# gongweibao/FleetX

Measured on AMD Instinct MI355X. Metric: tokens/sec (whole node) GPT-3 6.7B hybrid-parallel at 1/2/4/8 MI355X, higher is better.
Workload: dtype bf16; 1 GPU; model=gpt3-6.7B, global_batch=8, seq_len=1024, parallelism=dp1, micro_batch=8, hip_graph=True, grad_reduce_dtype=float32, recompute=False

## Files before the change

### csrc/kernels/bindings.cpp

```cpp
#include <hip/hip_runtime.h>
#include <pybind11/pybind11.h>
#include <pybind11/stl.h>
#include <stdint.h>
#include <string>
#include <stdexcept>
#include <vector>

namespace py = pybind11;
typedef uintptr_t ptr;

#include "fx_api.h"

#define P(x) reinterpret_cast<void*>(x)
#define CP(x) reinterpret_cast<const void*>(x)
#define S(x) reinterpret_cast<hipStream_t>(x)
#define F(x) reinterpret_cast<float*>(x)

static std::vector<long> v3(const std::vector<long>& a) {
  std::vector<long> r(a);
  r.resize(3, 0);
  return r;
}

PYBIND11_MODULE(_kernels, m) {
  m.doc() = "FleetX-AMD HIP kernels (gfx950)";
  m.def("coltile_splits", &fx_coltile_splits);
  m.def("add_ln_fwd", [](int dt, ptr x, ptr bias, ptr res, ptr g, ptr b, ptr s_out, ptr y,
                         ptr mean, ptr rstd, int rows, int h, float eps, float p, uint64_t key,
                         ptr salt, ptr st) {
    fx_add_ln_fwd(dt, CP(x), CP(bias), CP(res), CP(g), CP(b), P(s_out), P(y), F(mean), F(rstd),
                  rows, h, eps, p, key, CP(salt), S(st));
  });
  m.def("ln_bwd_row", [](int dt, ptr dy, ptr s, ptr mean, ptr rstd, ptr g, ptr ds_in, ptr ds_out,
                         ptr dx_out, int rows, int h, float p, uint64_t key, ptr salt, ptr st) {
    fx_ln_bwd_row(dt, CP(dy), CP(s), F(mean), F(rstd), CP(g), CP(ds_in), P(ds_out), P(dx_out),
                  rows, h, p, key, CP(salt), S(st));
  });
  m.def("ln_bwd_cols_blocks", &fx_ln_bwd_cols_blocks);
  m.def("ln_bwd_cols", [](int dt, ptr dy, ptr s, ptr mean, ptr rstd, ptr g, ptr ds_in, ptr ds_out,
                          ptr dx_out, int rows, int h, float p, uint64_t key, ptr part,
                          int with_dbias, ptr fg, ptr tg, int accg, ptr fb, ptr tb, int accb,
                          ptr fx, ptr tx, int accx, ptr salt, ptr st) {
    return fx_ln_bwd_cols(dt, CP(dy), CP(s), F(mean), F(rstd), CP(g), CP(ds_in), P(ds_out),
                          P(dx_out), rows, h, p, key, F(part), with_dbias, F(fg), P(tg), accg,
                          F(fb), P(tb), accb, F(fx), P(tx), accx, CP(salt), S(st));
  }, py::arg("dt"), py::arg("dy"), py::arg("s"), py::arg("mean"), py::arg("rstd"), py::arg("g"),
     py::arg("ds_in"), py::arg("ds_out"), py::arg("dx_out"), py::arg("rows"), py::arg("h"),
     py::arg("p"), py::arg("key"), py::arg("part"), py::arg("with_dbias"), py::arg("fg") = 0,
     py::arg("tg") = 0, py::arg("accg") = 0, py::arg("fb") = 0, py::arg("tb") = 0,
     py::arg("accb") = 0, py::arg("fx") = 0, py::arg("tx") = 0, py::arg("accx") = 0,
     py::arg("salt") = 0, py::arg("st") = 0);
  m.def("coltile_partial", [](int dt, int mode, ptr a, ptr b, ptr mean, ptr rstd, ptr p0, ptr p1,
                              int rows, int cols, int splits, ptr st, ptr cnt, ptr f0, ptr t0,
                              int acc0, ptr f1, ptr t1, int acc1) {
    fx_coltile_partial(dt, mode, CP(a), CP(b), F(mean), F(rstd), F(p0), F(p1), rows, cols, splits,
                       S(st), reinterpret_cast<int*>(cnt), F(f0), P(t0), acc0, F(f1), P(t1),
                       acc1);
  }, py::arg("dt"), py::arg("mode"), py::arg("a"), py::arg("b"), py::arg("mean"), py::arg("rstd"),
     py::arg("p0"), py::arg("p1"), py::arg("rows"), py::arg("cols"), py::arg("splits"),
     py::arg("st"), py::arg("cnt") = 0, py::arg("f0") = 0, py::arg("t0") = 0, py::arg("acc0") = 0,
     py::arg("f1") = 0, py::arg("t1") = 0, py::arg("acc1") = 0);
  m.def("coltile_finalize", [](int dt, ptr part, int splits, int cols, ptr out_f32, ptr out_t,
                               int accumulate, ptr st) {
    fx_coltile_finalize(dt, F(part), splits, cols, F(out_f32), P(out_t), accumulate, S(st));
  });
  m.def("bias_gelu_fwd", [](int dt, int erf, ptr x, ptr bias, ptr y, long n, int cols, ptr st) {
    fx_bias_gelu_fwd(dt, erf, CP(x), CP(bias), P(y), n, cols, S(st));
  });
  m.def("bias_gelu_bwd", [](int dt, int erf, ptr dy, ptr x, ptr bias, ptr dx, ptr part, int rows,
                            int cols, int splits, ptr st, ptr cnt, ptr out_f32, ptr out_t,
                            int acc) {
    fx_bias_gelu_bwd(dt, erf, CP(dy), CP(x), CP(bias), P(dx), F(part), rows, cols, splits, S(st),
                     reinterpret_cast<int*>(cnt), F(out_f32), P(out_t), acc);
  }, py::arg("dt"), py::arg("erf"), py::arg("dy"), py::arg("x"), py::arg("bias"), py::arg("dx"),
// ... 238 lines not shown
```

### csrc/kernels/fx_api.h

```cpp
#pragma once
#include <hip/hip_runtime.h>
#include <stdint.h>

extern "C" {
int fx_coltile_splits(int rows, int cols);
void fx_add_ln_fwd(int, const void*, const void*, const void*, const void*, const void*, void*,
                   void*, float*, float*, int, int, float, float, uint64_t, const void*,
                   hipStream_t);
void fx_ln_bwd_row(int, const void*, const void*, const float*, const float*, const void*,
                   const void*, void*, void*, int, int, float, uint64_t, const void*, hipStream_t);
int fx_ln_bwd_cols_blocks(int, int, int);
int fx_ln_bwd_cols(int, const void*, const void*, const float*, const float*, const void*,
                   const void*, void*, void*, int, int, float, uint64_t, float*, int, float*, void*,
                   int, float*, void*, int, float*, void*, int, const void*, hipStream_t);
void fx_coltile_partial(int, int, const void*, const void*, const float*, const float*, float*,
                        float*, int, int, int, hipStream_t, int*, float*, void*, int, float*,
                        void*, int);
void fx_coltile_finalize(int, const float*, int, int, float*, void*, int, hipStream_t);
void fx_bias_gelu_fwd(int, int, const void*, const void*, void*, long, int, hipStream_t);
void fx_bias_gelu_bwd(int, int, const void*, const void*, const void*, void*, float*, int, int, int,
                      hipStream_t, int*, float*, void*, int);
void fx_bias_dropout_add_fwd(int, const void*, const void*, const void*, void*, long, int, float,
                             uint64_t, const void*, hipStream_t);
void fx_dropout_bwd_colsum(int, const void*, void*, float*, int, int, int, float, uint64_t,
                           const void*, hipStream_t, int*, float*, void*, int);
void fx_dropout_fwd(int, const void*, void*, long, float, uint64_t, const void*, hipStream_t);
void fx_ce_stats(int, const void*, const int64_t*, int, int, long, float*, float*, float*, int,
                 hipStream_t);
void fx_ce_bwd(int, const void*, void*, const int64_t*, const float*, const float*, int, int, long,
               int, hipStream_t);
int fx_sumsq_blocks(long n);
void fx_sumsq_f32(const float*, long, float*, int, hipStream_t);
void fx_sumsq_16(int, const void*, long, float*, int, hipStream_t);
void fx_sumsq_chunks(const int64_t*, const int64_t*, int, float*, hipStream_t);
int fx_adamw(int dtype, int flags, void* master, const void* grad, float* m, float* v, void* p16,
             long n, float lr, float beta1, float beta2, float eps, float wd, float l2,
             const float* gscale, const int* skip, const int* step, const float* lr_dev,
// ... 75 lines not shown
```

### csrc/kernels/layout.hip

```cpp
#include "fx_api.h"
#include "fx_common.h"

namespace {

constexpr int TR = 64, TC = 256;
constexpr int TPAD = 2;

template <typename T, bool COLSUM>
__global__ __launch_bounds__(256) void transpose16_kernel(const uint16_t* __restrict__ x,
                                                          uint16_t* __restrict__ y,
                                                          float* __restrict__ part, int R, int C,
                                                          long ldx, long ldy, int tiles_c) {
  __shared__ uint16_t t[TR][TC + TPAD];
  const int bc = blockIdx.x % tiles_c;
  const int br = blockIdx.x / tiles_c;
  const int r0 = br * TR, c0 = bc * TC;
  const int tid = threadIdx.x;
  uint4 v[8];
#pragma unroll
  for (int k = 0; k < 8; ++k) {
    const int r = (tid >> 5) + 8 * k, cc = (tid & 31) * 8;
    if (r0 + r < R && c0 + cc < C)
      v[k] = *reinterpret_cast<const uint4*>(x + (long)(r0 + r) * ldx + c0 + cc);
    else
      v[k] = make_uint4(0, 0, 0, 0);
  }
#pragma unroll
  for (int k = 0; k < 8; ++k) {
    const int r = (tid >> 5) + 8 * k, cc = (tid & 31) * 8;
    uint32_t* d = reinterpret_cast<uint32_t*>(&t[r][cc]);
    d[0] = v[k].x;
    d[1] = v[k].y;
    d[2] = v[k].z;
    d[3] = v[k].w;
  }
  __syncthreads();
#pragma unroll
  for (int k = 0; k < 8; ++k) {
    const int id = tid + k * 256;
    const int c = id >> 3, rr = (id & 7) * 8;
    uint16_t h[8];
#pragma unroll
    for (int i = 0; i < 8; ++i) h[i] = t[rr + i][c];
    if (c0 + c < C && r0 + rr < R)
      *reinterpret_cast<uint4*>(y + (long)(c0 + c) * ldy + r0 + rr) =
          *reinterpret_cast<const uint4*>(h);
    if constexpr (COLSUM) {
      float s = 0.f;
#pragma unroll
      for (int i = 0; i < 8; ++i) s += Elt<T>::to_f(h[i]);
      s += __shfl_xor(s, 1, 64);
      s += __shfl_xor(s, 2, 64);
      s += __shfl_xor(s, 4, 64);
      if ((id & 7) == 0 && c0 + c < C) part[(long)br * C + c0 + c] = s;
    }
  }
}

}

extern "C" int fx_transpose16(int dtype, const void* x, void* y, float* part, int R, int C,
                              long ldx, long ldy, hipStream_t st) {
  if ((R | C) & 7 || ldx & 7 || ldy & 7) return -1;
  if (R == 0 || C == 0) return 0;
  const int tiles_c = (C + TC - 1) / TC;
  const long blocks = (long)tiles_c * ((R + TR - 1) / TR);
  if (blocks > 0x7fffffffL) return -2;
// ... 12 lines not shown
```

### csrc/kernels/norm_eltwise.hip

```cpp
#include "fx_api.h"
#include "fx_common.h"

namespace {

struct DropCfg {
  uint32_t klo, khi, thr;
  float scale;
  int enabled;
  const uint64_t* salt;
};

__device__ __forceinline__ DropCfg resolve_drop(DropCfg d) {
  if (d.enabled && d.salt != nullptr) {
    const uint64_t k = salt_key(((uint64_t)d.khi << 32) | d.klo, *d.salt);
    d.klo = (uint32_t)k;
    d.khi = (uint32_t)(k >> 32);
  }
  return d;
}

__device__ __forceinline__ float drop_apply(float v, uint64_t idx, const DropCfg& d) {
  if (!d.enabled) return v;
  uint32_t h = elem_rand_pair(idx, d.klo, d.khi);
  uint32_t r = (idx & 1) ? (h >> 16) : (h & 0xffffu);
  return r >= d.thr ? v * d.scale : 0.f;
}

__device__ __forceinline__ void drop_apply8(float* v, uint64_t idx0, const DropCfg& d) {
  if (!d.enabled) return;
#pragma unroll
  for (int q = 0; q < 4; ++q) {
    const uint32_t h = elem_rand_pair(idx0 + 2 * q, d.klo, d.khi);
// ... 195 lines not shown
#pragma unroll
    for (int i = 0; i < VPT; ++i) {
      const int c = (i * 64 + lane) * 8;
      dr[i] = make_uint4(0, 0, 0, 0);
      if (!MASK || c < h) dr[i] = *reinterpret_cast<const uint4*>(ds_in + base + c);
    }
  }
  const float m1 = wave_sum(s1) / h, m2 = wave_sum(s2) / h;
#pragma unroll
  for (int i = 0; i < VPT; ++i) {
    const int c = (i * 64 + lane) * 8;
    if (MASK && c >= h) continue;
    float o[8];
#pragma unroll
    for (int j = 0; j < 8; ++j) o[j] = rstd * (gdy[i][j] - m1 - xh[i][j] * m2);
    if (ds_in) {
      float r[8];
      unpack8<T>(dr[i], r);
#pragma unroll
      for (int j = 0; j < 8; ++j) o[j] += r[j];
    }
    store8<T>(ds_out + base + c, o);
    if (drop.enabled) {
      drop_apply8(o, base + c, drop);
      store8<T>(dx_out + base + c, o);
    } else if (dx_out != ds_out) {
      store8<T>(dx_out + base + c, o);
    }
  }
}

template <typename T>
__global__ __launch_bounds__(256) void ln_bwd_row_generic(
    const uint16_t* __restrict__ dy, const uint16_t* __restrict__ s,
    const float* __restrict__ mean_in, const float* __restrict__ rstd_in,
    const uint16_t* __restrict__ gamma, const uint16_t* __restrict__ ds_in,
    uint16_t* __restrict__ ds_out, uint16_t* __restrict__ dx_out, int rows, int h,
    DropCfg drop_) {
  const DropCfg drop = resolve_drop(drop_);
  const int lane = threadIdx.x & 63;
  const int row = blockIdx.x * 4 + (threadIdx.x >> 6);
  if (row >= rows) return;
  const size_t base = (size_t)row * h;
  const float mean = mean_in[row], rstd = rstd_in[row];
  const int nv = h / 8;
  float s1 = 0.f, s2 = 0.f;
// ... 3 lines not shown
    load8<T>(gamma + vi * 8, g);
    load8<T>(dy + base + vi * 8, d);
    for (int j = 0; j < 8; ++j) {
      float xh = (a[j] - mean) * rstd, gd = d[j] * g[j];
      s1 += gd;
      s2 += gd * xh;
    }
  }
  const float m1 = wave_sum(s1) / h, m2 = wave_sum(s2) / h;
  for (int vi = lane; vi < nv; vi += 64) {
    const int c = vi * 8;
    float a[8], g[8], d[8], o[8];
    load8<T>(s + base + c, a);
    load8<T>(gamma + c, g);
    load8<T>(dy + base + c, d);
    for (int j = 0; j < 8; ++j) o[j] = rstd * (d[j] * g[j] - m1 - (a[j] - mean) * rstd * m2);
    if (ds_in) {
      float r[8];
      load8<T>(ds_in + base + c, r);
      for (int j = 0; j < 8; ++j) o[j] += r[j];
    }
    store8<T>(ds_out + base + c, o);
    if (drop.enabled) {
      drop_apply8(o, base + c, drop);
      store8<T>(dx_out + base + c, o);
    } else if (dx_out != ds_out) {
      store8<T>(dx_out + base + c, o);
    }
  }
}

template <typename T, int VPT, int WPR, bool MASK, bool DB>
__global__ __launch_bounds__(256, 2) void ln_bwd_cols_kernel(
    const uint16_t* __restrict__ dy, const uint16_t* __restrict__ s,
    const float* __restrict__ mean_in, const float* __restrict__ rstd_in,
    const uint16_t* __restrict__ gamma, const uint16_t* __restrict__ ds_in,
    uint16_t* __restrict__ ds_out, uint16_t* __restrict__ dx_out, int rows, int h,
    int rows_per_group, float* __restrict__ part, DropCfg drop_) {
  constexpr int NG = 4 / WPR;
  __shared__ float red[4 * 512 * VPT];
  __shared__ float xs[2][4][2];
  const DropCfg drop = resolve_drop(drop_);
  const int lane = threadIdx.x & 63, w = threadIdx.x >> 6;
  const int grp = w / WPR, half = w % WPR;
  const int hw = h / WPR, cbase = half * hw;
  const int r0 = min(rows, (blockIdx.x * NG + grp) * rows_per_group);
// ... 70 lines not shown
        s2 += xs[k & 1][WPR * grp + q][1];
      }
    }
    if (!live) continue;
    const float m1 = s1 / h, m2 = s2 / h;
#pragma unroll
    for (int i = 0; i < VPT; ++i) {
      const int c = (i * 64 + lane) * 8;
      if (MASK && c >= hw) continue;
      float a[8], d[8], g[8], o[8];
      unpack8<T>(ca[i], a);
      unpack8<T>(cd[i], d);
      unpack8<T>(gp[i], g);
#pragma unroll
      for (int j = 0; j < 8; ++j) o[j] = rstd * (d[j] * g[j] - m1 - (a[j] - mean) * rstd * m2);
      if (ds_in) {
        float rr[8];
        unpack8<T>(cr[i], rr);
#pragma unroll
        for (int j = 0; j < 8; ++j) o[j] += rr[j];
      }
      store8<T>(ds_out + base + c, o);
      if (drop.enabled) {
        drop_apply8(o, base + c, drop);
        store8<T>(dx_out + base + c, o);
      } else if (dx_out != ds_out) {
        store8<T>(dx_out + base + c, o);
      }
      if (DB) {
#pragma unroll
        for (int j = 0; j < 8; ++j) ax[i][j] += round_to<T>(o[j]);
      }
    }
  }
#pragma unroll
  for (int arr = 0; arr < (DB ? 3 : 2); ++arr) {
    __syncthreads();
#pragma unroll
    for (int i = 0; i < VPT; ++i) {
      const int c = (i * 64 + lane) * 8;
      if (MASK && c >= hw) continue;
#pragma unroll
      for (int j = 0; j < 8; ++j)
        red[grp * h + cbase + c + j] = arr == 0 ? ag[i][j] : arr == 1 ? ab[i][j] : ax[DB ? i : 0][j];
    }
    __syncthreads();
// ... 241 lines not shown
  const int col = blockIdx.x * 128 + tx * 8;
  const int r0 = blockIdx.y * rows_per_split;
  const int r1 = min(rows, r0 + rows_per_split);
  float acc[8];
#pragma unroll
  for (int j = 0; j < 8; ++j) acc[j] = 0.f;
  if (col < cols) {
    float b[8];
    if (bias) load8<T>(bias + col, b);
    else {
#pragma unroll
      for (int j = 0; j < 8; ++j) b[j] = 0.f;
    }
    for (int r = r0 + ty; r < r1; r += 16) {
      const size_t off = (size_t)r * cols + col;
      float g[8], a[8];
      load8<T>(dy + off, g);
      load8<T>(x + off, a);
#pragma unroll
      for (int j = 0; j < 8; ++j) {
        float t = a[j] + b[j];
        g[j] *= ERF ? gelu_erf_grad(t) : gelu_tanh_grad(t);
      }
      store8<T>(dx + off, g);
#pragma unroll
      for (int j = 0; j < 8; ++j) acc[j] += round_to<T>(g[j]);
    }
  }
#pragma unroll
  for (int j = 0; j < 8; ++j) red[ty][tx * 8 + j] = acc[j];
  __syncthreads();
  if (threadIdx.x < 128) {
    float s = 0.f;
#pragma unroll
    for (int t = 0; t < 16; ++t) s += red[t][threadIdx.x];
    const int gc = blockIdx.x * 128 + threadIdx.x;
    if (part && gc < cols) st_part(part + (size_t)blockIdx.y * cols + gc, s);
  }
  if (fin.cnt) colsum_tail<T>(part, nullptr, cols, 1, fin);
}

template <typename T>
__global__ __launch_bounds__(256) void bias_dropout_add_fwd_kernel(
    const uint16_t* __restrict__ x, const uint16_t* __restrict__ bias,
    const uint16_t* __restrict__ residual, uint16_t* __restrict__ out, long n8, int cols,
    DropCfg drop_) {
// ... 85 lines not shown
                                                          DropCfg drop_) {
  const DropCfg drop = resolve_drop(drop_);
  const long n8 = n / 8;
  for (long v = blockIdx.x * (long)blockDim.x + threadIdx.x; v < n8; v += (long)gridDim.x * blockDim.x) {
    const long off = v * 8;
    float a[8];
    load8<T>(x + off, a);
    drop_apply8(a, (uint64_t)off, drop);
    store8<T>(y + off, a);
  }
  for (long i = n8 * 8 + blockIdx.x * (long)blockDim.x + threadIdx.x; i < n;
       i += (long)gridDim.x * blockDim.x)
    y[i] = Elt<T>::from_f(drop_apply(Elt<T>::to_f(x[i]), (uint64_t)i, drop));
}

DropCfg make_drop(float p, uint64_t key, const void* salt) {
  DropCfg d;
  d.enabled = p > 0.f ? 1 : 0;
  d.klo = (uint32_t)(key & 0xffffffffu);
  d.khi = (uint32_t)(key >> 32);
  d.thr = (uint32_t)(p * 65536.0f + 0.5f);
  d.scale = p < 1.f ? 1.f / (1.f - p) : 0.f;
  d.salt = reinterpret_cast<const uint64_t*>(salt);
  return d;
}

inline int grid_for(long n8) {
  long g = (n8 + 255) / 256;
  if (g > 8192) g = 8192;
  if (g < 1) g = 1;
  return (int)g;
}

inline int splits_for(int rows, int cols) {
  static const int blocks = [] {
    const char* e = getenv("FLEETX_COLSUM_BLOCKS");
    const int v = e ? atoi(e) : 0;
    return v > 0 ? v : 1024;
  }();
  int tiles = (cols + 127) / 128;
  int s = blocks / (tiles > 0 ? tiles : 1);
  if (s < 1) s = 1;
  int max_s = (rows + 15) / 16;
  if (s > max_s) s = max_s;
  if (s > 512) s = 512;
  return s;
// ... 48 lines not shown
                                 X, B, R, G, Be, S, Y, mean, rstd, rows, h, eps, d));
    }
  } else if (h % 8 == 0 && h < 8 * 512) {
#define LNM_CASE(V)                                                                          \
  case V:                                                                                    \
    FX_DISPATCH_T(dtype, add_ln_fwd_kernel<T, V, true><<<grid, block, 0, st>>>(              \
                             X, B, R, G, Be, S, Y, mean, rstd, rows, h, eps, d));            \
    break;
    switch ((h + 511) / 512) {
      LNM_CASE(1) LNM_CASE(2) LNM_CASE(3) LNM_CASE(4) LNM_CASE(5) LNM_CASE(6) LNM_CASE(7)
      LNM_CASE(8)
    }
#undef LNM_CASE
  } else {
    FX_DISPATCH_T(dtype, add_ln_fwd_generic<T><<<grid, block, 0, st>>>(
                             X, B, R, G, Be, S, Y, mean, rstd, rows, h, eps, d));
  }
#undef LN_CASE
}

extern "C" void fx_ln_bwd_row(int dtype, const void* dy, const void* s, const float* mean,
                              const float* rstd, const void* gamma, const void* ds_in,
                              void* ds_out, void* dx_out, int rows, int h, float p, uint64_t key,
                              const void* salt, hipStream_t st) {
  DropCfg d = make_drop(p, key, salt);
  dim3 grid((rows + 3) / 4), block(256);
  auto DY = (const uint16_t*)dy;
  auto S = (const uint16_t*)s;
  auto G = (const uint16_t*)gamma;
  auto DI = (const uint16_t*)ds_in;
  auto DS = (uint16_t*)ds_out;
  auto DX = (uint16_t*)dx_out;
#define LNB_CASE(V)                                                                       \
  case V:                                                                                 \
    FX_DISPATCH_T(dtype, ln_bwd_row_kernel<T, V><<<grid, block, 0, st>>>(                 \
                             DY, S, mean, rstd, G, DI, DS, DX, rows, h, d));              \
    break;
  if (h % 512 == 0 && h / 512 <= 8) {
    switch (h / 512) {
      LNB_CASE(1) LNB_CASE(2) LNB_CASE(3) LNB_CASE(4) LNB_CASE(5) LNB_CASE(6) LNB_CASE(7)
      LNB_CASE(8)
      default:
        FX_DISPATCH_T(dtype, ln_bwd_row_generic<T><<<grid, block, 0, st>>>(
                                 DY, S, mean, rstd, G, DI, DS, DX, rows, h, d));
    }
  } else if (h % 8 == 0 && h < 8 * 512) {
#define LNBM_CASE(V)                                                                      \
  case V:                                                                                 \
// ... 9 lines not shown
    FX_DISPATCH_T(dtype, ln_bwd_row_generic<T><<<grid, block, 0, st>>>(
                             DY, S, mean, rstd, G, DI, DS, DX, rows, h, d));
  }
#undef LNB_CASE
}

static int ln_cols_wpr(int h) { return h <= 1536 ? 1 : h <= 3072 ? 2 : 4; }
static int ln_cols_rows_per_group(int rows, int h) {
  const int ng = 4 / ln_cols_wpr(h);
  int rpg = (rows + 512 * ng - 1) / (512 * ng);
  return rpg < 2 ? 2 : rpg;
}
extern "C" int fx_ln_bwd_cols_blocks(int rows, int h, int max_h) {
  if (rows <= 0 || h > (max_h < 4096 ? max_h : 4096) || h % (8 * ln_cols_wpr(h))) return 0;
  const int ng = 4 / ln_cols_wpr(h), rpg = ln_cols_rows_per_group(rows, h);
  return (rows + ng * rpg - 1) / (ng * rpg);
}

extern "C" int fx_ln_bwd_cols(int dtype, const void* dy, const void* s, const float* mean,
                              const float* rstd, const void* gamma, const void* ds_in,
                              void* ds_out, void* dx_out, int rows, int h, float p, uint64_t key,
                              float* part, int with_dbias, float* fg, void* tg, int accg,
                              float* fb, void* tb, int accb, float* fx, void* tx, int accx,
                              const void* salt, hipStream_t st) {
  const int G = fx_ln_bwd_cols_blocks(rows, h, 4096);
  if (G == 0) return -1;
  const int wpr = ln_cols_wpr(h), hw = h / wpr;
  const int rpg = ln_cols_rows_per_group(rows, h);
  DropCfg d = make_drop(p, key, salt);
  auto DY = (const uint16_t*)dy;
  auto S = (const uint16_t*)s;
  auto GM = (const uint16_t*)gamma;
  auto DI = (const uint16_t*)ds_in;
  auto DS = (uint16_t*)ds_out;
  auto DX = (uint16_t*)dx_out;
  const int vpt = (hw + 511) / 512;
  const bool mask = hw % 512 != 0;
#define LNC_GO(V, W, M, DB)                                                                   \
  FX_DISPATCH_T(dtype, ln_bwd_cols_kernel<T, V, W, M, DB><<<G, 256, 0, st>>>(                 \
                           DY, S, mean, rstd, GM, DI, DS, DX, rows, h, rpg, part, d))
#define LNC_M(V, W)                                                                           \
  if (mask) {                                                                                 \
    if (with_dbias) { LNC_GO(V, W, true, true); } else { LNC_GO(V, W, true, false); }         \
  } else {                                                                                    \
    if (with_dbias) { LNC_GO(V, W, false, true); } else { LNC_GO(V, W, false, false); }       \
  }
#define LNC_V(V)                                                                              \
  case V:                                                                                     \
    if (wpr == 1) { LNC_M(V, 1) } else if (wpr == 2) { LNC_M(V, 2) } else { LNC_M(V, 4) }     \
    break;
  switch (vpt) {
    LNC_V(1) LNC_V(2) LNC_V(3)
// ... 99 lines not shown
```

### fleetx_amd/models/language_model/gpt/model.py

```python
import math

import torch
import torch.nn as nn

from .... import ops
from ....parallel import layers as L
from ....parallel import mappings as M
from ....parallel import topology as topo
from ....parallel.linear import fused_mlp
from ....parallel.recompute import recompute
from ....parallel.rng import get_rng_state_tracker


class GPTConfig:
    def __init__(self, vocab_size=50304, hidden_size=1024, num_layers=24, num_attention_heads=16,
                 ffn_hidden_size=None, hidden_dropout_prob=0.1, attention_probs_dropout_prob=0.1,
                 max_position_embeddings=1024, type_vocab_size=16, initializer_range=0.02,
                 use_recompute=False, recompute_granularity=None, sequence_parallel=False,
                 layer_norm_eps=1e-5, fused_linear=False, no_recompute_layers=None,
                 fused_lm_head_ce=False, dtype=torch.float32, **unused):
        self.vocab_size = vocab_size
        self.hidden_size = hidden_size
        self.num_layers = num_layers
        self.num_attention_heads = num_attention_heads
        self.ffn_hidden_size = ffn_hidden_size or 4 * hidden_size
        self.hidden_dropout_prob = hidden_dropout_prob
        self.attention_probs_dropout_prob = attention_probs_dropout_prob
        self.max_position_embeddings = max_position_embeddings
        self.type_vocab_size = type_vocab_size
        self.initializer_range = initializer_range
        self.use_recompute = use_recompute
        self.recompute_granularity = recompute_granularity or ("full" if use_recompute else None)
        self.sequence_parallel = sequence_parallel and topo.mp_world_size() > 1
        self.layer_norm_eps = layer_norm_eps
        self.no_recompute_layers = set(no_recompute_layers or [])
        self.dtype = dtype
        self.head_dim = hidden_size // num_attention_heads
        self.fused_lm_head_ce = bool(fused_lm_head_ce)

    @classmethod
    def from_model_config(cls, cfg, dtype=torch.float32):
        keys = ["vocab_size", "hidden_size", "num_layers", "num_attention_heads", "ffn_hidden_size",
                "hidden_dropout_prob", "attention_probs_dropout_prob", "max_position_embeddings",
                "type_vocab_size", "initializer_range", "use_recompute", "recompute_granularity",
                "sequence_parallel", "no_recompute_layers", "layer_norm_eps", "fused_lm_head_ce"]
        kw = {k: cfg[k] for k in keys if k in cfg and cfg[k] is not None}
        return cls(dtype=dtype, **kw)


def _key(stream):
    return get_rng_state_tracker().next_key(stream)


class GPTEmbeddings(nn.Module):
    def __init__(self, cfg):
        super().__init__()
        self.cfg = cfg
        self.word_embeddings = L.VocabParallelEmbedding(cfg.vocab_size, cfg.hidden_size,
                                                        std=cfg.initializer_range,
                                                        name="embeddings.word", dtype=cfg.dtype)
        self.position_embeddings = nn.Parameter(L.init_full_then_slice(
            (cfg.max_position_embeddings, cfg.hidden_size), cfg.initializer_range,
            "embeddings.position", dtype=cfg.dtype))
        self.position_embeddings.sequence_parallel = cfg.sequence_parallel

    def forward(self, input_ids, position_ids=None):
        b, s = input_ids.shape
        if position_ids is None:
# ... 64 lines not shown

class GPTMLP(nn.Module):
    def __init__(self, cfg, idx):
        super().__init__()
        std = cfg.initializer_range
        self.fc1 = L.ColumnParallelLinear(cfg.hidden_size, cfg.ffn_hidden_size, bias=True,
                                          skip_bias_add=True,
                                          sequence_parallel=cfg.sequence_parallel, std=std,
                                          name="layers.%d.mlp.fc1" % idx, dtype=cfg.dtype)
        self.fc2 = L.RowParallelLinear(cfg.ffn_hidden_size, cfg.hidden_size, bias=True,
                                       skip_bias_add=True, sequence_parallel=cfg.sequence_parallel,
                                       std=std, name="layers.%d.mlp.fc2" % idx, dtype=cfg.dtype)
        self.fc1.sp_chunk_major = self.fc2.sp_chunk_major = bool(cfg.sequence_parallel)

    def forward(self, x):
        if topo.mp_world_size() == 1 and type(self.fc1) is L.ColumnParallelLinear \
                and type(self.fc2) is L.RowParallelLinear:
            return fused_mlp(x, self.fc1.weight, self.fc1.bias, self.fc2.weight), self.fc2.bias
        y, b = self.fc1(x)
        y = ops.bias_gelu(y, b, approximate=True)
        return self.fc2(y)


class GPTDecoderLayer(nn.Module):

    def __init__(self, cfg, idx):
        super().__init__()
        self.cfg = cfg
        self.idx = idx
        self.ln1 = ops.FusedLayerNorm(cfg.hidden_size, cfg.layer_norm_eps, dtype=cfg.dtype)
        self.attn = GPTAttention(cfg, idx)
        self.ln2 = ops.FusedLayerNorm(cfg.hidden_size, cfg.layer_norm_eps, dtype=cfg.dtype)
        self.mlp = GPTMLP(cfg, idx)
        if cfg.sequence_parallel:
            L.mark_sequence_parallel(self.ln1)
            L.mark_sequence_parallel(self.ln2)

    def _attn_block(self, x):
        return self.attn(self.ln1(x))

    def _attn_block_out(self, x):
        return self._attn_block(x)[0]

    def _forward(self, x):
        cfg = self.cfg
        p = cfg.hidden_dropout_prob if self.training else 0.0
        stream = "local_seed" if cfg.sequence_parallel else "global_seed"
        if cfg.recompute_granularity == "full_attn" and self.training:
            a, ab = recompute(self._attn_block_out, x), self.attn.out_proj.bias
        else:
            x, h1 = ops.layer_norm_keep_input(x, self.ln1.weight, self.ln1.bias, self.ln1.eps)
            a, ab = self.attn(h1)
        k1 = _key(stream) if p > 0 else 0
        x2, h2 = ops.add_layer_norm(a, ab, x, self.ln2.weight, self.ln2.bias, self.ln2.eps, p, k1)
        m, mb = self.mlp(h2)
        k2 = _key(stream) if p > 0 else 0
        return ops.bias_dropout_add(m, mb, x2, p, k2)

    def forward(self, x):
        if (self.cfg.recompute_granularity == "full" and self.training
                and self.idx not in self.cfg.no_recompute_layers):
            return recompute(self._forward, x)
        return self._forward(x)


class GPTModel(nn.Module):

    def __init__(self, cfg, layer_range=None, has_embedding=True, has_final_ln=True):
        super().__init__()
        self.cfg = cfg
        start, end = layer_range if layer_range is not None else (0, cfg.num_layers)
        self.embeddings = GPTEmbeddings(cfg) if has_embedding else None
        self.layers = nn.ModuleList([GPTDecoderLayer(cfg, i) for i in range(start, end)])
        self.final_ln = ops.FusedLayerNorm(cfg.hidden_size, cfg.layer_norm_eps,
                                           dtype=cfg.dtype) if has_final_ln else None
        if has_final_ln and cfg.sequence_parallel:
            L.mark_sequence_parallel(self.final_ln)

    def forward(self, input_ids=None, position_ids=None, hidden=None):
        x = self.embeddings(input_ids, position_ids) if self.embeddings is not None else hidden
        for layer in self.layers:
            x = layer(x)
        if self.final_ln is not None:
            x = self.final_ln(x)
        return x


class GPTForPretraining(nn.Module):

    def __init__(self, cfg):
        super().__init__()
        self.cfg = cfg
        self.gpt = GPTModel(cfg)
        emb = self.gpt.embeddings
        if emb is not None:
            emb.word_embeddings.weight._fx_fused_wgrad_ok = True
            emb.word_embeddings.weight._fx_grad_parts = 2
            emb.position_embeddings._fx_fused_wgrad_ok = True

    def forward(self, input_ids, position_ids=None):
        h = self.gpt(input_ids, position_ids)
        w = self.gpt.embeddings.word_embeddings.weight
        if self.cfg.fused_lm_head_ce and self.training:
            return L.parallel_lm_head_input(h, w, sequence_parallel=self.cfg.sequence_parallel)
        logits = L.parallel_lm_logits(h, w, parallel_output=True,
# ... 40 lines not shown
```

### fleetx_amd/ops/norm.py

```python
import os

import torch

from . import _lib
from ..parallel import grad_sink as sink, rng as _rng


_TICKETS = {}


def colsum_tickets(device, cols):
    st = torch.cuda.current_stream(device).cuda_stream
    need = 32 * ((cols + 127) // 128)
    t = _TICKETS.get(st)
    if t is None or t.numel() < need:
        t = torch.zeros(max(4096, need), dtype=torch.int32, device=device)
        _TICKETS[st] = t
    return t.data_ptr()


_TARGET_KW = (("f0", "t0", "acc0"), ("f1", "t1", "acc1"))


def _coltile(mode, x, aux, rows, cols, targets):
# ... 34 lines not shown
    if not _lib.vec8_ok(cols, x):
        sink.store_or_add(dst, x.reshape(-1, cols).float().sum(0).view_as(dst), accumulate)
        return dst
    if dst.dtype != torch.float32 or not dst.is_contiguous():
        raise ValueError("col_sum_f32: dst must be contiguous fp32")
    _coltile(1, x, (0, 0, 0), x.numel() // cols, cols, [(dst.data_ptr(), 0, int(accumulate))])
    return dst


def _dropout_ref(x, p, key):
    if p <= 0.0:
        return x
    m = _rng.keep_mask(x.shape, p, key, x.device)
    return torch.where(m, x * (1.0 / (1.0 - p)), torch.zeros_like(x))


def _ln_bwd_cols_max_h():
    mode = os.environ.get("FLEETX_LN_BWD_FUSED", "1")
    return {"0": 0, "2": 4096}.get(mode, 1536)


def _ln_bwd_cols(k, dc, dy, s, mean, rstd, weight, ctx, ds_in, ds, dx, rows, h):
    G = k.ln_bwd_cols_blocks(rows, h, 4096)
    with_db = bool(ctx.has_bias)
    part = torch.empty(3 if with_db else 2, G, h, device=dy.device, dtype=torch.float32)
    prms = (weight, ctx.lnbias, ctx.bias if with_db else None)
    outs, grads = [], []
    for prm in prms:
        t, g = ((0, 0, 0), None) if prm is None else \
            _col_target(prm, sink.fused(prm, fp32_contiguous=True), h, dy)
        outs.append(t)
        grads.append(g)
    (fg, tg, ag), (fb, tb, ab), (fx, tx, ax) = outs
    rc = k.ln_bwd_cols(dc, dy.data_ptr(), s.data_ptr(), mean.data_ptr(), rstd.data_ptr(),
                       weight.data_ptr(), _lib.ptr(ds_in), ds.data_ptr(), dx.data_ptr(), rows, h,
                       float(ctx.p), ctx.key, part.data_ptr(), int(with_db), fg, tg, ag, fb, tb,
                       ab, fx, tx, ax, _rng.device_salt_ptr(), _lib.stream())
    if rc != 0:
        raise RuntimeError("ln_bwd_cols: shape rows=%d h=%d not covered" % (rows, h))
    for prm, (f32, _, _) in zip(prms, outs):
        if f32:
            sink.close_write(prm)
    return grads


class _AddLayerNorm(torch.autograd.Function):
    @staticmethod
    def forward(ctx, x, bias, residual, weight, lnbias, eps, p, key, store_sum):
        h = x.shape[-1]
        rows = x.numel() // h
        ctx.p, ctx.key, ctx.has_bias, ctx.has_res = p, key, bias is not None, residual is not None
        ctx.h = h
        x = x.contiguous()
        if _lib.vec8_ok(h, x, bias, residual, weight, lnbias):
            k = _lib.kernels()
            fused = bias is not None or residual is not None or p > 0
            s = torch.empty_like(x) if fused else None
            y = torch.empty_like(x)
            mean = torch.empty(rows, device=x.device, dtype=torch.float32)
            rstd = torch.empty_like(mean)
            k.add_ln_fwd(_lib.dt_code(x.dtype), x.data_ptr(), _lib.ptr(bias), _lib.ptr(residual),
                         weight.data_ptr(), lnbias.data_ptr(), _lib.ptr(s), y.data_ptr(),
                         mean.data_ptr(), rstd.data_ptr(), rows, h, float(eps), float(p), key,
                         _rng.device_salt_ptr(), _lib.stream())
            s_saved = s if s is not None else x
            if s is None and store_sum:
                s = x
        else:
            v = x
            if bias is not None or residual is not None or p > 0:
                v = x.float() if bias is None else x.float() + bias.float()
                v = _dropout_ref(v, p, key)
                if residual is not None:
                    v = v + residual.float()
# ... 2 lines not shown
            s = v if (store_sum or bias is not None or residual is not None or p > 0) else None
            vf = v.float()
            mean = vf.mean(-1).reshape(-1)
            var = ((vf - mean.view(*vf.shape[:-1], 1)) ** 2).mean(-1).reshape(-1)
            rstd = torch.rsqrt(var + eps)
            y = ((vf - mean.view(*vf.shape[:-1], 1)) * rstd.view(*vf.shape[:-1], 1) * weight.float()
                 + lnbias.float()).to(x.dtype)
        ctx.save_for_backward(s_saved, mean, rstd, weight)
        ctx.lnbias, ctx.bias = lnbias, bias
        ctx.return_sum = s is not None
        if s is None:
            return y
        return s, y

    @staticmethod
    def backward(ctx, *grads):
        if ctx.return_sum:
            ds_in, dy = grads
        else:
            ds_in, dy = None, grads[0]
        s, mean, rstd, weight = ctx.saved_tensors
        h = ctx.h
        rows = s.numel() // h
        dy = dy.contiguous()
        if ds_in is not None:
            ds_in = ds_in.contiguous()
        if _lib.vec8_ok(h, dy, ds_in, s, weight):
            k = _lib.kernels()
            dc = _lib.dt_code(dy.dtype)
            ds = torch.empty_like(dy)
            dx = torch.empty_like(dy) if ctx.p > 0 else ds
            if k.ln_bwd_cols_blocks(rows, h, _ln_bwd_cols_max_h()) > 0:
                dw, db, dbias = _ln_bwd_cols(k, dc, dy, s, mean, rstd, weight, ctx, ds_in, ds, dx,
                                             rows, h)
                dres = ds if ctx.has_res else None
                return dx, dbias, dres, dw, db, None, None, None, None
            k.ln_bwd_row(dc, dy.data_ptr(), s.data_ptr(), mean.data_ptr(), rstd.data_ptr(),
                         weight.data_ptr(), _lib.ptr(ds_in), ds.data_ptr(), dx.data_ptr(), rows, h,
                         float(ctx.p), ctx.key, _rng.device_salt_ptr(), _lib.stream())
            direct = sink.fused(weight) and sink.fused(ctx.lnbias)
            (tw, dw), (tb, db) = (_col_target(prm, direct, h, dy) for prm in (weight, ctx.lnbias))
            _coltile(0, dy, (s.data_ptr(), mean.data_ptr(), rstd.data_ptr()), rows, h, [tw, tb])
            if direct:
                sink.close_write(weight)
                sink.close_write(ctx.lnbias)
            dbias = None
            if ctx.has_bias:
                if sink.fused(ctx.bias):
                    mg, acc = sink.open_write(ctx.bias)
                    col_sum_f32(dx, mg, acc)
                    sink.close_write(ctx.bias)
                else:
                    dbias = col_sum(dx, h)
        else:
            sf = s.float().reshape(rows, h)
            xh = (sf - mean.view(rows, 1)) * rstd.view(rows, 1)
            g = dy.float().reshape(rows, h) * weight.float()
            m1 = g.mean(-1, keepdim=True)
            m2 = (g * xh).mean(-1, keepdim=True)
            dsf = rstd.view(rows, 1) * (g - m1 - xh * m2)
            if ds_in is not None:
                dsf = dsf + ds_in.float().reshape(rows, h)
            ds = dsf.to(dy.dtype).reshape(dy.shape)
            dx = _dropout_ref(ds, ctx.p, ctx.key)
            dw = sink.deliver(weight, (dy.float().reshape(rows, h) * xh).sum(0), weight.dtype,
                              on_gpu=True)
            db = sink.deliver(ctx.lnbias, dy.float().reshape(rows, h).sum(0), weight.dtype,
                              on_gpu=True)
            dbias = None
            if ctx.has_bias:
                dbias = sink.deliver(ctx.bias, dx.float().reshape(rows, h).sum(0), dy.dtype,
                                     on_gpu=True)
        dres = ds if ctx.has_res else None
        return dx, dbias, dres, dw, db, None, None, None, None


def add_layer_norm(x, bias, residual, weight, lnbias, eps=1e-5, p=0.0, key=0):
    return _AddLayerNorm.apply(x, bias, residual, weight, lnbias, eps, p, key, True)


def layer_norm(x, weight, bias, eps=1e-5):
    return _AddLayerNorm.apply(x, None, None, weight, bias, eps, 0.0, 0, False)


def layer_norm_keep_input(x, weight, bias, eps=1e-5):
    return _AddLayerNorm.apply(x, None, None, weight, bias, eps, 0.0, 0, True)


class FusedLayerNorm(torch.nn.Module):

    def __init__(self, hidden, eps=1e-5, dtype=None, device=None):
        super().__init__()
        self.weight = torch.nn.Parameter(torch.ones(hidden, dtype=dtype, device=device))
        self.bias = torch.nn.Parameter(torch.zeros(hidden, dtype=dtype, device=device))
        self.weight._fx_fused_wgrad_ok = True
        self.bias._fx_fused_wgrad_ok = True
        self.eps = eps
        self.normalized_shape = (hidden,)

    def forward(self, x):
        return layer_norm(x, self.weight, self.bias, self.eps)
# ... 1 lines not shown
```

Baseline: 28370 tokens/s.

## Fuse layer-boundary bias-dropout-add into next layer's LayerNorm

Each decoder layer can now hand off its final bias+dropout+residual add as a pending sum, so the next layer's ln1 (or the final LN) runs as a fused add_layer_norm instead of a separate bias_dropout_add followed by layer_norm. This removes one elementwise kernel and one full activation read/write per layer boundary in forward and backward. The backward adds a rounding option on ds before dropout to match the unfused numerics, and computes the bias gradient separately in the chained case. A transpose kernel also gains a fast path without bounds checks for full tiles.

After: 28340 tokens/s. Within noise of the previous version (-0.1%).

```diff
diff --git a/csrc/kernels/bindings.cpp b/csrc/kernels/bindings.cpp
--- a/csrc/kernels/bindings.cpp
+++ b/csrc/kernels/bindings.cpp
@@ -32,24 +32,27 @@
                   rows, h, eps, p, key, CP(salt), S(st));
   });
   m.def("ln_bwd_row", [](int dt, ptr dy, ptr s, ptr mean, ptr rstd, ptr g, ptr ds_in, ptr ds_out,
-                         ptr dx_out, int rows, int h, float p, uint64_t key, ptr salt, ptr st) {
+                         ptr dx_out, int rows, int h, float p, uint64_t key, ptr salt, ptr st,
+                         int round_ds) {
     fx_ln_bwd_row(dt, CP(dy), CP(s), F(mean), F(rstd), CP(g), CP(ds_in), P(ds_out), P(dx_out),
-                  rows, h, p, key, CP(salt), S(st));
-  });
+                  rows, h, p, key, CP(salt), S(st), round_ds);
+  }, py::arg("dt"), py::arg("dy"), py::arg("s"), py::arg("mean"), py::arg("rstd"), py::arg("g"),
+     py::arg("ds_in"), py::arg("ds_out"), py::arg("dx_out"), py::arg("rows"), py::arg("h"),
+     py::arg("p"), py::arg("key"), py::arg("salt"), py::arg("st"), py::arg("round_ds") = 0);
   m.def("ln_bwd_cols_blocks", &fx_ln_bwd_cols_blocks);
   m.def("ln_bwd_cols", [](int dt, ptr dy, ptr s, ptr mean, ptr rstd, ptr g, ptr ds_in, ptr ds_out,
                           ptr dx_out, int rows, int h, float p, uint64_t key, ptr part,
                           int with_dbias, ptr fg, ptr tg, int accg, ptr fb, ptr tb, int accb,
-                          ptr fx, ptr tx, int accx, ptr salt, ptr st) {
+                          ptr fx, ptr tx, int accx, ptr salt, ptr st, int round_ds) {
     return fx_ln_bwd_cols(dt, CP(dy), CP(s), F(mean), F(rstd), CP(g), CP(ds_in), P(ds_out),
                           P(dx_out), rows, h, p, key, F(part), with_dbias, F(fg), P(tg), accg,
-                          F(fb), P(tb), accb, F(fx), P(tx), accx, CP(salt), S(st));
+                          F(fb), P(tb), accb, F(fx), P(tx), accx, CP(salt), S(st), round_ds);
   }, py::arg("dt"), py::arg("dy"), py::arg("s"), py::arg("mean"), py::arg("rstd"), py::arg("g"),
      py::arg("ds_in"), py::arg("ds_out"), py::arg("dx_out"), py::arg("rows"), py::arg("h"),
      py::arg("p"), py::arg("key"), py::arg("part"), py::arg("with_dbias"), py::arg("fg") = 0,
      py::arg("tg") = 0, py::arg("accg") = 0, py::arg("fb") = 0, py::arg("tb") = 0,
      py::arg("accb") = 0, py::arg("fx") = 0, py::arg("tx") = 0, py::arg("accx") = 0,
-     py::arg("salt") = 0, py::arg("st") = 0);
+     py::arg("salt") = 0, py::arg("st") = 0, py::arg("round_ds") = 0);
   m.def("coltile_partial", [](int dt, int mode, ptr a, ptr b, ptr mean, ptr rstd, ptr p0, ptr p1,
                               int rows, int cols, int splits, ptr st, ptr cnt, ptr f0, ptr t0,
                               int acc0, ptr f1, ptr t1, int acc1) {
diff --git a/csrc/kernels/fx_api.h b/csrc/kernels/fx_api.h
--- a/csrc/kernels/fx_api.h
+++ b/csrc/kernels/fx_api.h
@@ -8,11 +8,12 @@
                    void*, float*, float*, int, int, float, float, uint64_t, const void*,
                    hipStream_t);
 void fx_ln_bwd_row(int, const void*, const void*, const float*, const float*, const void*,
-                   const void*, void*, void*, int, int, float, uint64_t, const void*, hipStream_t);
+                   const void*, void*, void*, int, int, float, uint64_t, const void*, hipStream_t,
+                   int);
 int fx_ln_bwd_cols_blocks(int, int, int);
 int fx_ln_bwd_cols(int, const void*, const void*, const float*, const float*, const void*,
                    const void*, void*, void*, int, int, float, uint64_t, float*, int, float*, void*,
-                   int, float*, void*, int, float*, void*, int, const void*, hipStream_t);
+                   int, float*, void*, int, float*, void*, int, const void*, hipStream_t, int);
 void fx_coltile_partial(int, int, const void*, const void*, const float*, const float*, float*,
                         float*, int, int, int, hipStream_t, int*, float*, void*, int, float*,
                         void*, int);
diff --git a/csrc/kernels/layout.hip b/csrc/kernels/layout.hip
--- a/csrc/kernels/layout.hip
+++ b/csrc/kernels/layout.hip
@@ -16,14 +16,21 @@
   const int br = blockIdx.x / tiles_c;
   const int r0 = br * TR, c0 = bc * TC;
   const int tid = threadIdx.x;
+  const bool whole = r0 + TR <= R && c0 + TC <= C;
   uint4 v[8];
+  if (whole) {
+    const uint16_t* xp = x + (long)(r0 + (tid >> 5)) * ldx + c0 + (tid & 31) * 8;
 #pragma unroll
-  for (int k = 0; k < 8; ++k) {
-    const int r = (tid >> 5) + 8 * k, cc = (tid & 31) * 8;
-    if (r0 + r < R && c0 + cc < C)
-      v[k] = *reinterpret_cast<const uint4*>(x + (long)(r0 + r) * ldx + c0 + cc);
-    else
-      v[k] = make_uint4(0, 0, 0, 0);
+    for (int k = 0; k < 8; ++k) v[k] = *reinterpret_cast<const uint4*>(xp + 8 * k * ldx);
+  } else {
+#pragma unroll
+    for (int k = 0; k < 8; ++k) {
+      const int r = (tid >> 5) + 8 * k, cc = (tid & 31) * 8;
+      if (r0 + r < R && c0 + cc < C)
+        v[k] = *reinterpret_cast<const uint4*>(x + (long)(r0 + r) * ldx + c0 + cc);
+      else
+        v[k] = make_uint4(0, 0, 0, 0);
+    }
   }
 #pragma unroll
   for (int k = 0; k < 8; ++k) {
@@ -42,7 +49,7 @@
     uint16_t h[8];
 #pragma unroll
     for (int i = 0; i < 8; ++i) h[i] = t[rr + i][c];
-    if (c0 + c < C && r0 + rr < R)
+    if (whole || (c0 + c < C && r0 + rr < R))
       *reinterpret_cast<uint4*>(y + (long)(c0 + c) * ldy + r0 + rr) =
           *reinterpret_cast<const uint4*>(h);
     if constexpr (COLSUM) {
diff --git a/csrc/kernels/norm_eltwise.hip b/csrc/kernels/norm_eltwise.hip
--- a/csrc/kernels/norm_eltwise.hip
+++ b/csrc/kernels/norm_eltwise.hip
@@ -8,6 +8,7 @@
   float scale;
   int enabled;
   const uint64_t* salt;
+  int round_in;
 };
 
 __device__ __forceinline__ DropCfg resolve_drop(DropCfg d) {
@@ -249,6 +250,10 @@
     }
     store8<T>(ds_out + base + c, o);
     if (drop.enabled) {
+      if (drop.round_in) {
+#pragma unroll
+        for (int j = 0; j < 8; ++j) o[j] = round_to<T>(o[j]);
+      }
       drop_apply8(o, base + c, drop);
       store8<T>(dx_out + base + c, o);
     } else if (dx_out != ds_out) {
@@ -298,6 +303,10 @@
     }
     store8<T>(ds_out + base + c, o);
     if (drop.enabled) {
+      if (drop.round_in) {
+#pragma unroll
+        for (int j = 0; j < 8; ++j) o[j] = round_to<T>(o[j]);
+      }
       drop_apply8(o, base + c, drop);
       store8<T>(dx_out + base + c, o);
     } else if (dx_out != ds_out) {
@@ -414,6 +423,10 @@
       }
       store8<T>(ds_out + base + c, o);
       if (drop.enabled) {
+        if (drop.round_in) {
+#pragma unroll
+          for (int j = 0; j < 8; ++j) o[j] = round_to<T>(o[j]);
+        }
         drop_apply8(o, base + c, drop);
         store8<T>(dx_out + base + c, o);
       } else if (dx_out != ds_out) {
@@ -701,6 +714,10 @@
         float t = a[j] + b[j];
         g[j] *= ERF ? gelu_erf_grad(t) : gelu_tanh_grad(t);
       }
+      if constexpr (__is_same(T, f16)) {
+#pragma unroll
+        for (int j = 0; j < 8; ++j) asm volatile("" : "+v"(g[j]));
+      }
       store8<T>(dx + off, g);
 #pragma unroll
       for (int j = 0; j < 8; ++j) acc[j] += round_to<T>(g[j]);
@@ -832,6 +849,7 @@
   d.thr = (uint32_t)(p * 65536.0f + 0.5f);
   d.scale = p < 1.f ? 1.f / (1.f - p) : 0.f;
   d.salt = reinterpret_cast<const uint64_t*>(salt);
+  d.round_in = 0;
   return d;
 }
 
@@ -926,8 +944,9 @@
 extern "C" void fx_ln_bwd_row(int dtype, const void* dy, const void* s, const float* mean,
                               const float* rstd, const void* gamma, const void* ds_in,
                               void* ds_out, void* dx_out, int rows, int h, float p, uint64_t key,
-                              const void* salt, hipStream_t st) {
+                              const void* salt, hipStream_t st, int round_ds) {
   DropCfg d = make_drop(p, key, salt);
+  d.round_in = round_ds;
   dim3 grid((rows + 3) / 4), block(256);
   auto DY = (const uint16_t*)dy;
   auto S = (const uint16_t*)s;
@@ -983,12 +1002,13 @@
                               void* ds_out, void* dx_out, int rows, int h, float p, uint64_t key,
                               float* part, int with_dbias, float* fg, void* tg, int accg,
                               float* fb, void* tb, int accb, float* fx, void* tx, int accx,
-                              const void* salt, hipStream_t st) {
+                              const void* salt, hipStream_t st, int round_ds) {
   const int G = fx_ln_bwd_cols_blocks(rows, h, 4096);
   if (G == 0) return -1;
   const int wpr = ln_cols_wpr(h), hw = h / wpr;
   const int rpg = ln_cols_rows_per_group(rows, h);
   DropCfg d = make_drop(p, key, salt);
+  d.round_in = round_ds;
   auto DY = (const uint16_t*)dy;
   auto S = (const uint16_t*)s;
   auto GM = (const uint16_t*)gamma;
diff --git a/fleetx_amd/models/language_model/gpt/model.py b/fleetx_amd/models/language_model/gpt/model.py
--- a/fleetx_amd/models/language_model/gpt/model.py
+++ b/fleetx_amd/models/language_model/gpt/model.py
@@ -18,7 +18,8 @@
                  max_position_embeddings=1024, type_vocab_size=16, initializer_range=0.02,
                  use_recompute=False, recompute_granularity=None, sequence_parallel=False,
                  layer_norm_eps=1e-5, fused_linear=False, no_recompute_layers=None,
-                 fused_lm_head_ce=False, dtype=torch.float32, **unused):
+                 fused_lm_head_ce=False, fuse_layer_boundary=True, dtype=torch.float32,
+                 **unused):
         self.vocab_size = vocab_size
         self.hidden_size = hidden_size
         self.num_layers = num_layers
@@ -37,13 +38,15 @@
         self.dtype = dtype
         self.head_dim = hidden_size // num_attention_heads
         self.fused_lm_head_ce = bool(fused_lm_head_ce)
+        self.fuse_layer_boundary = bool(fuse_layer_boundary)
 
     @classmethod
     def from_model_config(cls, cfg, dtype=torch.float32):
         keys = ["vocab_size", "hidden_size", "num_layers", "num_attention_heads", "ffn_hidden_size",
                 "hidden_dropout_prob", "attention_probs_dropout_prob", "max_position_embeddings",
                 "type_vocab_size", "initializer_range", "use_recompute", "recompute_granularity",
-                "sequence_parallel", "no_recompute_layers", "layer_norm_eps", "fused_lm_head_ce"]
+                "sequence_parallel", "no_recompute_layers", "layer_norm_eps", "fused_lm_head_ce",
+                "fuse_layer_boundary"]
         kw = {k: cfg[k] for k in keys if k in cfg and cfg[k] is not None}
         return cls(dtype=dtype, **kw)
 
@@ -154,6 +157,23 @@
         return self.fc2(y)
 
 
+class PendingSum:
+
+    def __init__(self, m, bias, res, p, key):
+        self.m, self.bias, self.res, self.p, self.key = m, bias, res, p, key
+
+    def resolve(self):
+        return ops.bias_dropout_add(self.m, self.bias, self.res, self.p, self.key)
+
+    def layer_norm(self, ln):
+        return ops.add_layer_norm(self.m, self.bias, self.res, ln.weight, ln.bias, ln.eps,
+                                  self.p, self.key, chained=True)
+
+
+def _hooked(module):
+    return bool(module._forward_hooks)
+
+
 class GPTDecoderLayer(nn.Module):
 
     def __init__(self, cfg, idx):
@@ -174,12 +194,17 @@
     def _attn_block_out(self, x):
         return self._attn_block(x)[0]
 
-    def _forward(self, x):
+    def _forward(self, x, hand_on=False):
         cfg = self.cfg
         p = cfg.hidden_dropout_prob if self.training else 0.0
         stream = "local_seed" if cfg.sequence_parallel else "global_seed"
         if cfg.recompute_granularity == "full_attn" and self.training:
+            if isinstance(x, PendingSum):
+                x = x.resolve()
             a, ab = recompute(self._attn_block_out, x), self.attn.out_proj.bias
+        elif isinstance(x, PendingSum):
+            x, h1 = x.layer_norm(self.ln1)
+            a, ab = self.attn(h1)
         else:
             x, h1 = ops.layer_norm_keep_input(x, self.ln1.weight, self.ln1.bias, self.ln1.eps)
             a, ab = self.attn(h1)
@@ -187,13 +212,17 @@
         x2, h2 = ops.add_layer_norm(a, ab, x, self.ln2.weight, self.ln2.bias, self.ln2.eps, p, k1)
         m, mb = self.mlp(h2)
         k2 = _key(stream) if p > 0 else 0
+        if hand_on:
+            return PendingSum(m, mb, x2, p, k2)
         return ops.bias_dropout_add(m, mb, x2, p, k2)
 
-    def forward(self, x):
+    def forward(self, x, hand_on=False):
         if (self.cfg.recompute_granularity == "full" and self.training
                 and self.idx not in self.cfg.no_recompute_layers):
+            if isinstance(x, PendingSum):
+                x = x.resolve()
             return recompute(self._forward, x)
-        return self._forward(x)
+        return self._forward(x, hand_on)
 
 
 class GPTModel(nn.Module):
@@ -211,8 +240,13 @@
 
     def forward(self, input_ids=None, position_ids=None, hidden=None):
         x = self.embeddings(input_ids, position_ids) if self.embeddings is not None else hidden
-        for layer in self.layers:
-            x = layer(x)
+        fuse = self.cfg.fuse_layer_boundary and self.training
+        last = len(self.layers) - 1
+        for i, layer in enumerate(self.layers):
+            x = layer(x, hand_on=fuse and (i < last or self.final_ln is not None)
+                      and not _hooked(layer))
+        if isinstance(x, PendingSum):
+            return x.layer_norm(self.final_ln)[1]
         if self.final_ln is not None:
             x = self.final_ln(x)
         return x
diff --git a/fleetx_amd/ops/norm.py b/fleetx_amd/ops/norm.py
--- a/fleetx_amd/ops/norm.py
+++ b/fleetx_amd/ops/norm.py
@@ -80,7 +80,7 @@
 
 def _ln_bwd_cols(k, dc, dy, s, mean, rstd, weight, ctx, ds_in, ds, dx, rows, h):
     G = k.ln_bwd_cols_blocks(rows, h, 4096)
-    with_db = bool(ctx.has_bias)
+    with_db = bool(ctx.has_bias) and not ctx.chained
     part = torch.empty(3 if with_db else 2, G, h, device=dy.device, dtype=torch.float32)
     prms = (weight, ctx.lnbias, ctx.bias if with_db else None)
     outs, grads = [], []
@@ -93,7 +93,8 @@
     rc = k.ln_bwd_cols(dc, dy.data_ptr(), s.data_ptr(), mean.data_ptr(), rstd.data_ptr(),
                        weight.data_ptr(), _lib.ptr(ds_in), ds.data_ptr(), dx.data_ptr(), rows, h,
                        float(ctx.p), ctx.key, part.data_ptr(), int(with_db), fg, tg, ag, fb, tb,
-                       ab, fx, tx, ax, _rng.device_salt_ptr(), _lib.stream())
+                       ab, fx, tx, ax, _rng.device_salt_ptr(), _lib.stream(),
+                       round_ds=int(ctx.chained))
     if rc != 0:
         raise RuntimeError("ln_bwd_cols: shape rows=%d h=%d not covered" % (rows, h))
     for prm, (f32, _, _) in zip(prms, outs):
@@ -102,12 +103,24 @@
     return grads
 
 
+def _bias_grad(bias, dx, h):
+    if sink.fused(bias):
+        mg, acc = sink.open_write(bias)
+        col_sum_f32(dx, mg, acc)
+        sink.close_write(bias)
+        return None
+    return col_sum(dx, h)
+
+
 class _AddLayerNorm(torch.autograd.Function):
     @staticmethod
-    def forward(ctx, x, bias, residual, weight, lnbias, eps, p, key, store_sum):
+    def forward(ctx, x, bias, residual, weight, lnbias, eps, p, key, store_sum, chained=False):
         h = x.shape[-1]
         rows = x.numel() // h
         ctx.p, ctx.key, ctx.has_bias, ctx.has_res = p, key, bias is not None, residual is not None
+        ctx.chained = bool(chained)
+        if chained:
+            ctx.set_materialize_grads(False)
         ctx.h = h
         x = x.contiguous()
         if _lib.vec8_ok(h, x, bias, residual, weight, lnbias):
@@ -156,7 +169,7 @@
         s, mean, rstd, weight = ctx.saved_tensors
         h = ctx.h
         rows = s.numel() // h
-        dy = dy.contiguous()
+        dy = dy.contiguous() if dy is not None else torch.zeros_like(s)
         if ds_in is not None:
             ds_in = ds_in.contiguous()
         if _lib.vec8_ok(h, dy, ds_in, s, weight):
@@ -167,25 +180,21 @@
             if k.ln_bwd_cols_blocks(rows, h, _ln_bwd_cols_max_h()) > 0:
                 dw, db, dbias = _ln_bwd_cols(k, dc, dy, s, mean, rstd, weight, ctx, ds_in, ds, dx,
                                              rows, h)
+                if ctx.has_bias and ctx.chained:
+                    dbias = _bias_grad(ctx.bias, dx, h)
                 dres = ds if ctx.has_res else None
-                return dx, dbias, dres, dw, db, None, None, None, None
+                return dx, dbias, dres, dw, db, None, None, None, None, None
             k.ln_bwd_row(dc, dy.data_ptr(), s.data_ptr(), mean.data_ptr(), rstd.data_ptr(),
                          weight.data_ptr(), _lib.ptr(ds_in), ds.data_ptr(), dx.data_ptr(), rows, h,
-                         float(ctx.p), ctx.key, _rng.device_salt_ptr(), _lib.stream())
+                         float(ctx.p), ctx.key, _rng.device_salt_ptr(), _lib.stream(),
+                         round_ds=int(ctx.chained))
             direct = sink.fused(weight) and sink.fused(ctx.lnbias)
             (tw, dw), (tb, db) = (_col_target(prm, direct, h, dy) for prm in (weight, ctx.lnbias))
             _coltile(0, dy, (s.data_ptr(), mean.data_ptr(), rstd.data_ptr()), rows, h, [tw, tb])
             if direct:
                 sink.close_write(weight)
                 sink.close_write(ctx.lnbias)
-            dbias = None
-            if ctx.has_bias:
-                if sink.fused(ctx.bias):
-                    mg, acc = sink.open_write(ctx.bias)
-                    col_sum_f32(dx, mg, acc)
-                    sink.close_write(ctx.bias)
-                else:
-                    dbias = col_sum(dx, h)
+            dbias = _bias_grad(ctx.bias, dx, h) if ctx.has_bias else None
         else:
             sf = s.float().reshape(rows, h)
             xh = (sf - mean.view(rows, 1)) * rstd.view(rows, 1)
@@ -206,11 +215,11 @@
                 dbias = sink.deliver(ctx.bias, dx.float().reshape(rows, h).sum(0), dy.dtype,
                                      on_gpu=True)
         dres = ds if ctx.has_res else None
-        return dx, dbias, dres, dw, db, None, None, None, None
-
-
-def add_layer_norm(x, bias, residual, weight, lnbias, eps=1e-5, p=0.0, key=0):
-    return _AddLayerNorm.apply(x, bias, residual, weight, lnbias, eps, p, key, True)
+        return dx, dbias, dres, dw, db, None, None, None, None, None
+
+
+def add_layer_norm(x, bias, residual, weight, lnbias, eps=1e-5, p=0.0, key=0, chained=False):
+    return _AddLayerNorm.apply(x, bias, residual, weight, lnbias, eps, p, key, True, chained)
 
 
 def layer_norm(x, weight, bias, eps=1e-5):
```
